# zdule/distributed_learning

Measured on AMD Instinct MI355X. Metric: images/sec (whole node) ResNet-50 synthetic ImageNet, higher is better.
Workload: dtype bf16

## Files before the change

### csrc/include/dla_kernels.h

```cpp
#pragma once

#include <hip/hip_runtime.h>
#include <stdint.h>

#include "dla_dtype.h"
#include "dla_lists.h"

namespace dla {

struct SgdParams {
  float lr;
  float momentum;
  float dampening;
  float weight_decay;
  float grad_scale;
  int nesterov;
  int first_step;
};

void launch_sgd_ema_list(const SgdList& list, const EmaSlots& ema, const float* omd, int nblocks, int grad_dtype,
                         bool use_momentum, const SgdParams& hp, hipStream_t stream);
void launch_ema_update_list(const EmaList& list, int nblocks, const float* omd, hipStream_t stream);
void launch_ema_swap_list(const EmaList& list, int nblocks, hipStream_t stream);
void launch_sgd_list(const SgdList& list, int nblocks, int grad_dtype, bool use_momentum, const SgdParams& hp,
// ... 256 lines not shown
void launch_gemm_nt_splitk(const void* A, int64_t lda, const void* B, int64_t ldb, bool b_kmajor, float* partial,
                           int splits, void* C, int M, int N, int K, const void* addend, int64_t ld_addend,
                           hipStream_t stream);

int conv3x3_stats_rows(int64_t P, int Cout, int tile = kTileAuto, int K = 0, bool wide_ok = true);
int pick_conv_tile(int64_t P, int N, int tile, int K, bool wide_ok);
bool halo_conv_eligible(int Cin, int Cout, int W, int stride, bool fwd);
void launch_conv3x3_halo(const void* x, const void* w, void* y, int N, int H, int W, float* stats,
                         hipStream_t stream, const void* addend = nullptr);
void launch_conv3x3_fwd(const void* x, const void* w, void* y, int N, int H, int W, int Cin, int Cout, int stride,
                        float* stats, hipStream_t stream, int tile = kTileAuto);
void launch_conv3x3_dgrad(const void* dy, const void* w, void* dx, int N, int H, int W, int Cin, int Cout,
                          const void* addend, hipStream_t stream, int tile = kTileAuto,
                          const BnBwdArgs* bn_bwd = nullptr);
void launch_conv3x3s2_dgrad(const void* dy, const void* w, void* dx, int N, int H, int W, int Cin, int Cout,
                            hipStream_t stream);
int stem_stats_rows(int64_t P, int Cout = 64);
int stem_stream_rows(int64_t P, int Cout);
bool launch_stem_stream(const void* xs, const void* wpk, void* y, int N, int BH, int BW, float* stats,
                        hipStream_t stream);
void set_stem_stream(int mode);

void launch_stem_fold(const void* x, void* xs, int N, int H, int W, hipStream_t stream);
void launch_stem_fwd(const void* xs, const void* wpk, void* y, int N, int H, int W, int Cout, float* stats,
                     hipStream_t stream);
int stem_wgrad_splits(int N, int H, int W, int Cout);
void launch_stem_wgrad(const void* dy, const void* xs, float* partial, int splits, void* dwpk, int out_dtype, int N,
                       int H, int W, int Cout, hipStream_t stream);
bool stem_wgrad_bn_eligible(int N, int H, int W, int Cout, int OH, int OW);
int stem_wgrad_bn_splits(int N, int H, int W);
void launch_stem_wgrad_bn(const void* dy_pool, const uint8_t* pos, const void* x, const float* ws, const void* xs,
// ... 13 lines not shown
```

### csrc/include/dla_mfma.h

```cpp
#pragma once

#include "dla_common.h"

namespace dla {
namespace mm {

typedef __bf16 bf16x8_t __attribute__((ext_vector_type(8)));
typedef float f32x4_t __attribute__((ext_vector_type(4)));
typedef short s16x4_t __attribute__((ext_vector_type(4)));

struct FastDiv {
  uint32_t d, m_lo, m_hi;
};
__host__ __device__ inline FastDiv make_fastdiv(uint32_t d) {
  const uint64_t m = ((1ull << 40) + d - 1) / d;
  return FastDiv{d, (uint32_t)m, (uint32_t)(m >> 32)};
}
__device__ __forceinline__ uint32_t fdiv(uint32_t n, const FastDiv& f) {
  return (__umulhi(n, f.m_lo) + n * f.m_hi) >> 8;
}

constexpr int kThreads = 256;
#ifndef DLA_RM_SWIZZLE
#define DLA_RM_SWIZZLE 1
// ... 307 lines not shown
    } else {
      kr = kk * 16 + 8 * (g >> 1) + q;
      cn = r0 + 16 * (g & 1) + 4 * p;
    }
    return tr_frag(s + tr_off<W>(kr, cn), s + tr_off<W>(kr + 4, cn));
  } else {
    if constexpr (DLA_RM_SWIZZLE) {
      const int r = r0 + (lane & (kMS - 1)), lc = kk * (kKS / 8) + lane / kMS;
      return *reinterpret_cast<const bf16x8_t*>(s + r * kBK + ((lc ^ ((r >> 1) & 7)) << 3));
    }
    return *reinterpret_cast<const bf16x8_t*>(s + (r0 + (lane & (kMS - 1))) * (kBK + 8) + kk * kKS +
                                              8 * (lane / kMS));
  }
}

template <int BM, int BN, int NT, bool kT = false, class LA, class LB>
__device__ __forceinline__ void mainloop(const LA& la, const LB& lb, int kbeg, int kend, Acc<BM, BN, NT>& acc,
                                         char* smem) {
  static_assert(LA::kNT == NT && LB::kNT == NT, "loaders built for another block size");
  using GA = TileGeom<BM, NT>;
  using GB = TileGeom<BN, NT>;
  using AC = Acc<BM, BN, NT>;
  constexpr int WM = AC::WM, WN = AC::WN, TM = AC::TM, TN = AC::TN;
  bf16_t* As = reinterpret_cast<bf16_t*>(smem);
  bf16_t* Bs = As + (LA::kKMajor ? GA::kKElems : GA::kRowElems);
  const int wid = threadIdx.x >> 6, wr = wid / AC::WGN, wc = wid % AC::WGN;
  ushort8_t ra[GA::CH], rb[GB::CH];
  auto gload = [&](int k0) {
#pragma unroll
    for (int i = 0; i < GA::CH; ++i) ra[i] = la.load(i, k0);
#pragma unroll
    for (int i = 0; i < GB::CH; ++i) rb[i] = lb.load(i, k0);
  };
  const int nk = (kend - kbeg + kBK - 1) / kBK;
  if (nk <= 0) return;
  gload(kbeg);
  tile_store<BM, LA>(As, ra);
  tile_store<BN, LB>(Bs, rb);
  __syncthreads();
  for (int t = 0; t < nk; ++t) {
    if (t + 1 < nk) gload(kbeg + (t + 1) * kBK);
#pragma unroll
    for (int kk = 0; kk < kBK / kKS; ++kk) {
      bf16x8_t af[TM], bfr[TN];
#pragma unroll
      for (int i = 0; i < TM; ++i) af[i] = tile_frag<BM, LA>(As, wr * WM + i * kMS, kk);
#pragma unroll
      for (int j = 0; j < TN; ++j) bfr[j] = tile_frag<BN, LB>(Bs, wc * WN + j * kMS, kk);
#pragma unroll
      for (int i = 0; i < TM; ++i)
#pragma unroll
        for (int j = 0; j < TN; ++j) acc.v[i][j] = mfma_t<kT>(af[i], bfr[j], acc.v[i][j]);
    }
    __syncthreads();
    if (t + 1 < nk) {
      tile_store<BM, LA>(As, ra);
// ... 8 lines not shown
  const int r = r0 + (lane & (kMS - 1)), lc = kk * (kKS / 8) + lane / kMS;
  return *reinterpret_cast<const bf16x8_t*>(s + r * kBK + ((lc ^ ((r >> 1) & 7)) << 3));
}

template <int W, class L>
__device__ __forceinline__ bf16x8_t glds_frag(const bf16_t* s, int r0, int kk) {
  if constexpr (L::kKMajor) return tile_frag<W, L>(s, r0, kk);
  else return rm_glds_frag(s, r0, kk);
}

template <int BM, int BN, int NS>
__host__ __device__ constexpr size_t glds_lds_bytes() {
  return (size_t)NS * (BM + BN) * kBK * sizeof(bf16_t);
}

template <int BM, int BN, int NT, int NS, bool kT = false, class LA, class LB>
__device__ __forceinline__ void mainloop_glds(const LA& la, const LB& lb, int kbeg, int kend, Acc<BM, BN, NT>& acc,
                                              char* smem) {
  static_assert(NS == 2 || NS == 3, "2 or 3 stages");
  static_assert(LA::kNT == NT && LB::kNT == NT, "loaders built for another block size");
  using GA = TileGeom<BM, NT>;
  using GB = TileGeom<BN, NT>;
  using AC = Acc<BM, BN, NT>;
  constexpr int L = GA::CH + GB::CH;
  constexpr int WM = AC::WM, WN = AC::WN, TM = AC::TM, TN = AC::TN;
  constexpr int SA = BM * kBK, SB = BN * kBK;
  bf16_t* base = reinterpret_cast<bf16_t*>(smem);
  const int wave = threadIdx.x >> 6, wr = wave / AC::WGN, wc = wave % AC::WGN;
  const uint32_t lds0 = lds_addr(smem);
  const uint32_t wofs = (uint32_t)__builtin_amdgcn_readfirstlane(wave * 64 * 16);
  const int nk = (kend - kbeg + kBK - 1) / kBK;
  if (nk <= 0) return;
  LA pa = la;
  LB pb = lb;
  pa.prep();
  pb.prep();
  auto issue = [&](int t) {
    const int st = t % NS;
    const int k0 = kbeg + t * kBK;
    const uint32_t a_base = lds0 + (uint32_t)(st * (SA + SB)) * 2u + wofs;
    const uint32_t b_base = a_base + (uint32_t)SA * 2u;
#pragma unroll
    for (int i = 0; i < GA::CH; ++i) glds16(pa.src(i, k0), a_base + (uint32_t)(i * NT * 16));
#pragma unroll
    for (int i = 0; i < GB::CH; ++i) glds16(pb.src(i, k0), b_base + (uint32_t)(i * NT * 16));
  };
#pragma unroll
  for (int p = 0; p < NS - 1; ++p)
    if (p < nk) issue(p);
  for (int t = 0; t < nk; ++t) {
    if constexpr (NS == 3) {
      if (t + 1 < nk) vm_wait<L>();
      else vm_wait<0>();
    } else {
// ... 46 lines not shown
    bf16x8_t af[TM], bfr[TN];
#pragma unroll
    for (int i = 0; i < TM; ++i) af[i] = glds_frag<BM, LA>(As, wr * WM + i * kMS, kk);
#pragma unroll
    for (int j = 0; j < TN; ++j) bfr[j] = glds_frag<BN, LB>(Bs, wc * WN + j * kMS, kk);
    __builtin_amdgcn_s_setprio(1);
#pragma unroll
    for (int i = 0; i < TM; ++i)
#pragma unroll
      for (int j = 0; j < TN; ++j) acc.v[i][j] = mfma_t<kT>(af[i], bfr[j], acc.v[i][j]);
    __builtin_amdgcn_s_setprio(0);
    if (kk == 0) mid();
  }
}

template <int BM, int BN, int NT, int NS, bool kT = false, class LA, class LB>
__device__ __forceinline__ void mainloop_glds2(const LA& la, const LB& lb, int kbeg, int kend, Acc<BM, BN, NT>& acc,
                                               char* smem) {
  static_assert(NS == 2 || NS == 3, "2 or 3 stages");
  static_assert(LA::kNT == NT && LB::kNT == NT, "loaders built for another block size");
  using GA = TileGeom<BM, NT>;
  using GB = TileGeom<BN, NT>;
  using AC = Acc<BM, BN, NT>;
  constexpr int L = GA::CH + GB::CH;
  constexpr int WM = AC::WM, WN = AC::WN, TM = AC::TM, TN = AC::TN;
  constexpr int SA = BM * kBK, SB = BN * kBK;
  bf16_t* base = reinterpret_cast<bf16_t*>(smem);
  const int wave = threadIdx.x >> 6, wr = wave / AC::WGN, wc = wave % AC::WGN;
  const uint32_t lds0 = lds_addr(smem);
  const uint32_t wofs = (uint32_t)__builtin_amdgcn_readfirstlane(wave * 64 * 16);
  const int nk = (kend - kbeg + kBK - 1) / kBK;
  if (nk <= 0) return;
  LA pa = la;
  LB pb = lb;
  pa.prep();
  pb.prep();
  auto issue_a = [&](int t) {
    const int k0 = kbeg + t * kBK;
    loader_step(pa, k0, 0);
    const uint32_t a_base = lds0 + (uint32_t)((t % NS) * (SA + SB)) * 2u + wofs;
#pragma unroll
    for (int i = 0; i < GA::CH; ++i) glds16(loader_src(pa, i, k0, 0), a_base + (uint32_t)(i * NT * 16));
  };
  auto issue_b = [&](int t) {
    const int k0 = kbeg + t * kBK;
    loader_step(pb, k0, 0);
    const uint32_t b_base = lds0 + (uint32_t)((t % NS) * (SA + SB) + SA) * 2u + wofs;
#pragma unroll
    for (int i = 0; i < GB::CH; ++i) glds16(loader_src(pb, i, k0, 0), b_base + (uint32_t)(i * NT * 16));
  };
#pragma unroll
  for (int p = 0; p < NS - 1; ++p)
    if (p < nk) {
      issue_a(p);
      issue_b(p);
    }
  for (int t = 0; t < nk; ++t) {
    if constexpr (NS == 3) {
      if (t + 1 < nk) vm_wait<L>();
      else vm_wait<0>();
// ... 16 lines not shown

template <class L, int W, int NT>
__device__ __forceinline__ void bissue(const L& l, int k0, uint32_t lds) {
  constexpr int CH = TileGeom<W, NT>::CH;
  uint32_t vo[CH];
  if (l.bcheck(k0)) {
#pragma unroll
    for (int i = 0; i < CH; ++i) vo[i] = l.bvoff_chk(i, k0);
  } else {
#pragma unroll
    for (int i = 0; i < CH; ++i) vo[i] = l.bvo[i];
  }
  bglds<CH, NT * 16>(vo, l.bsrd, (uint32_t)__builtin_amdgcn_readfirstlane(l.bsoff(k0)), lds);
}

template <int BM, int BN, int NT, int NS, bool kT = false, class LA, class LB>
__device__ __forceinline__ void mainloop_bglds(const LA& la, const LB& lb, int kbeg, int kend, Acc<BM, BN, NT>& acc,
                                               char* smem) {
  static_assert(NS == 2 || NS == 3, "2 or 3 stages");
  static_assert(LA::kNT == NT && LB::kNT == NT, "loaders built for another block size");
  using GA = TileGeom<BM, NT>;
  using GB = TileGeom<BN, NT>;
  using AC = Acc<BM, BN, NT>;
  constexpr int L = GA::CH + GB::CH;
  constexpr int WM = AC::WM, WN = AC::WN, TM = AC::TM, TN = AC::TN;
  constexpr int SA = BM * kBK, SB = BN * kBK;
  bf16_t* base = reinterpret_cast<bf16_t*>(smem);
  const int wave = threadIdx.x >> 6, wr = wave / AC::WGN, wc = wave % AC::WGN;
  const uint32_t lds0 = lds_addr(smem);
  const uint32_t wofs = (uint32_t)__builtin_amdgcn_readfirstlane(wave * 64 * 16);
  const int nk = (kend - kbeg + kBK - 1) / kBK;
  if (nk <= 0) return;
  LA pa = la;
  LB pb = lb;
  pa.prep();
  pb.prep();
  pa.bprep();
  pb.bprep();
  auto issue_a = [&](int t) {
    const int k0 = kbeg + t * kBK;
    loader_step(pa, k0, 0);
    bissue<LA, BM, NT>(pa, k0, lds0 + (uint32_t)((t % NS) * (SA + SB)) * 2u + wofs);
  };
  auto issue_b = [&](int t) {
    const int k0 = kbeg + t * kBK;
    loader_step(pb, k0, 0);
    bissue<LB, BN, NT>(pb, k0, lds0 + (uint32_t)((t % NS) * (SA + SB) + SA) * 2u + wofs);
  };
#pragma unroll
  for (int p = 0; p < NS - 1; ++p)
    if (p < nk) {
      issue_a(p);
      issue_b(p);
    }
  for (int t = 0; t < nk; ++t) {
    if constexpr (NS == 3) {
      if (t + 1 < nk) vm_wait<L>();
      else vm_wait<0>();
    } else {
      vm_wait<0>();
    }
    asm volatile("s_waitcnt lgkmcnt(0)" ::: "memory");
    __builtin_amdgcn_s_barrier();
    asm volatile("" ::: "memory");
    const bool more = t + NS - 1 < nk;
    if (more) issue_a(t + NS - 1);
    const bf16_t* As = base + (t % NS) * (SA + SB);
    const bf16_t* Bs = As + SA;
    kstep_mfma<BM, BN, NT, LA, LB, kT>(As, Bs, wr, wc, acc, [&] {
      if (more) issue_b(t + NS - 1);
    });
  }
  __syncthreads();
}

template <int PIPE, bool kT = false, int BM, int BN, int NT, class LA, class LB>
__device__ __forceinline__ void run_mainloop(const LA& la, const LB& lb, int kbeg, int kend, Acc<BM, BN, NT>& acc,
                                             char* smem) {
  if constexpr (PIPE == 0) mainloop<BM, BN, NT, kT>(la, lb, kbeg, kend, acc, smem);
  else if constexpr (PIPE >= 6) mainloop_bglds<BM, BN, NT, PIPE - 4, kT>(la, lb, kbeg, kend, acc, smem);
  else if constexpr (PIPE >= 4) mainloop_glds2<BM, BN, NT, PIPE - 2, kT>(la, lb, kbeg, kend, acc, smem);
  else mainloop_glds<BM, BN, NT, PIPE, kT>(la, lb, kbeg, kend, acc, smem);
}

template <int PIPE, int BM, int BN, class LA, class LB>
__host__ __device__ constexpr size_t run_mainloop_lds_bytes() {
  return PIPE == 0 ? mainloop_lds_bytes<BM, BN, LA, LB>()
                   : glds_lds_bytes<BM, BN, (PIPE >= 6 ? PIPE - 4 : (PIPE >= 4 ? PIPE - 2 : PIPE))>();
}

template <int BM, int BN, bool kStats, int NT = kThreads>
__host__ __device__ constexpr size_t epilogue_lds_bytes() {
  return (size_t)BM * (BN + 8) * sizeof(bf16_t) > (size_t)NT * 64 ? (size_t)BM * (BN + 8) * sizeof(bf16_t)
                                                                  : (size_t)NT * 64;
}

template <int BM, int BN, int NT = kThreads>
// ... 386 lines not shown
```

### csrc/kernels/conv.hip

```cpp
#include "dla_common.h"
#include "dla_kernels.h"
#include "dla_knob.h"
#include "dla_mfma.h"

#include <algorithm>
#include <cstdlib>
#include <type_traits>

namespace dla {

using namespace mm;

struct ConvGeom {
  int N, H, W, Cin;
  int OH, OW, Cout;
  int stride;
  FastDiv fOW, fOH;
};

template <int W, bool kFlip, int NT = kThreads>
struct Im2colRowLoader {
  static constexpr bool kKMajor = false;
  static constexpr int kNT = NT;
  static constexpr int CH = TileGeom<W, NT>::CH;
  const bf16_t* x;
  int H, Wd, C;
// ... 408 lines not shown
  }
  __device__ const void* src(int i, int k0) const {
    const int c = threadIdx.x + i * NT, kr = c / TileGeom<W>::KPR;
    const int p = k0 + kr;
    if (p >= kend || kh[i] < 0) return zero_src();
    const uint32_t q = fdiv((uint32_t)p, g.fOW);
    const int ow = p - (int)q * g.OW;
    const uint32_t n = fdiv(q, g.fOH);
    const int oh = (int)q - (int)n * g.OH;
    const int ih = oh * g.stride - 1 + kh[i], iw = ow * g.stride - 1 + kw[i];
    if ((unsigned)ih >= (unsigned)g.H || (unsigned)iw >= (unsigned)g.W) return zero_src();
    return x + (((int64_t)n * g.H + ih) * g.W + iw) * g.Cin + ci[i];
  }
};

template <int BM, int BN, bool kStats, int PIPE, int NT>
__global__ __launch_bounds__(NT, blocks_per_cu(BM, BN, NT)) void conv3x3_fwd_kernel(const bf16_t* __restrict__ x,
                                                                  const bf16_t* __restrict__ w,
                                                                  bf16_t* __restrict__ y, ConvGeom g,
                                                                  float* __restrict__ stats) {
  extern __shared__ __attribute__((aligned(16))) char smem_raw[];
  const int64_t P = (int64_t)g.N * g.OH * g.OW;
  const int nbn = (g.Cout + BN - 1) / BN;
  const int tile = xcd_remap(blockIdx.x, gridDim.x);
  const int bm = tile / nbn, bn = tile % nbn;
  const int64_t row0 = (int64_t)bm * BM;
  const int col0 = bn * BN;
  const int K = 9 * g.Cin;
  constexpr bool kAny = PIPE >= 100;
  const RowLoader<BN, NT> lb{w, K, (int64_t)col0, g.Cout, K};
  std::conditional_t<kAny, Im2colRowLoaderAnyC<BM, false, NT>, Im2colRowLoader<BM, false, NT>> la{
      x, g.H, g.W, g.Cin, g.stride};
  la.init(g, row0, P, g.OH, g.OW, g.fOW, g.fOH);
  ColStats<BM, BN, NT> st;
  st.zero();
  Acc<BM, BN, NT> acc;
  acc.zero();
  run_mainloop<PIPE % 100>(la, lb, 0, K, acc, smem_raw);
  epilogue_bf16<BM, BN, kStats, false, NT>(acc, y, g.Cout, P, g.Cout, row0, col0, st, nullptr, 0, smem_raw);
  if constexpr (kStats) stats_flush<BM, BN, NT>(st, stats + (int64_t)bm * g.Cout * 2, g.Cout, col0, smem_raw);
}

template <int BM, int BN, int PIPE, int NT>
__global__ __launch_bounds__(NT, blocks_per_cu(BM, BN, NT)) void conv3x3_dgrad_kernel(const bf16_t* __restrict__ dy,
                                                                    const bf16_t* __restrict__ w,
                                                                    bf16_t* __restrict__ dx, ConvGeom g,
                                                                    const bf16_t* __restrict__ addend, BnBwdEpi bnb) {
  extern __shared__ __attribute__((aligned(16))) char smem_raw[];
  const int64_t P = (int64_t)g.N * g.H * g.W;
  const int nbn = (g.Cin + BN - 1) / BN;
  const int tile = xcd_remap(blockIdx.x, gridDim.x);
  const int bm = tile / nbn, bn = tile % nbn;
  const int64_t row0 = (int64_t)bm * BM;
  const int col0 = bn * BN;
  const int K = 9 * g.Cout;
  constexpr bool kAny = PIPE >= 100;
  std::conditional_t<kAny, WeightTapKLoaderAnyC<BN, NT>, WeightTapKLoader<BN, NT>> lb{w, g.Cout, g.Cin, col0};
  if constexpr (kAny) lb.prep();
  std::conditional_t<kAny, Im2colRowLoaderAnyC<BM, true, NT>, Im2colRowLoader<BM, true, NT>> la{dy, g.OH, g.OW,
                                                                                                 g.Cout, 1};
  la.init(g, row0, P, g.H, g.W, g.fOW, g.fOH);
  ColStats<BM, BN, NT> st;
  Acc<BM, BN, NT> acc;
  acc.zero();
  run_mainloop<PIPE % 100>(la, lb, 0, K, acc, smem_raw);
  epilogue_bf16<BM, BN, false, true, NT>(acc, dx, g.Cin, P, g.Cin, row0, col0, st, addend, g.Cin, smem_raw, &bnb, bm);
}

template <int BM, int BN, int PIPE, int NT = kThreads>
__global__ __launch_bounds__(NT, blocks_per_cu(BM, BN, NT)) void conv3x3s2_dgrad_kernel(const bf16_t* __restrict__ dy,
                                                                                      const bf16_t* __restrict__ w,
                                                                                      bf16_t* __restrict__ dx,
                                                                                      ConvGeom g) {
  extern __shared__ __attribute__((aligned(16))) char smem_raw[];
  const int64_t P = (int64_t)g.N * g.OH * g.OW;
  const int nbn = (g.Cin + BN - 1) / BN;
  const int per_class = (int)((P + BM - 1) / BM) * nbn;
  const int cls_slot = blockIdx.x / per_class;
  const S2Class cls{cls_slot < 2 ? 1 : 0, (cls_slot & 1) == 0 ? 1 : 0};
  const int tile = xcd_remap(blockIdx.x - cls_slot * per_class, per_class);
  const int bm = tile / nbn, bn = tile % nbn;
  const int64_t row0 = (int64_t)bm * BM;
  const int col0 = bn * BN;
  const int K = cls.ntaps() * g.Cout;
  const S2WeightKLoader<BN, NT> lb{w, g.Cout, g.Cin, col0, cls};
  S2DgradRowLoader<BM, NT> la{dy, g.OH, g.OW, g.Cout, cls};
  la.init(row0, P, g.fOW, g.fOH);
  ColStats<BM, BN, NT> st;
  Acc<BM, BN, NT> acc;
  acc.zero();
  run_mainloop<PIPE>(la, lb, 0, K, acc, smem_raw);
  const S2RowMap rm{g.OH, g.OW, cls.ph, cls.pw, g.fOW, g.fOH};
  epilogue_bf16<BM, BN, false, false, NT, S2RowMap>(acc, dx, g.Cin, P, g.Cin, row0, col0, st, nullptr, 0,
                                                   smem_raw, nullptr, 0, rm);
}

template <int BM, int BN, int PIPE, int NT = kThreads>
__global__ __launch_bounds__(NT, blocks_per_cu(BM, BN, NT)) void conv3x3_wgrad_kernel(const bf16_t* __restrict__ dy,
                                                                                    const bf16_t* __restrict__ x,
                                                                                    ConvGeom g, float* __restrict__ part,
                                                                                    int k_per_split, int ntiles,
                                                                                    int remap) {
  extern __shared__ __attribute__((aligned(16))) char smem_raw[];
  const int P = g.N * g.OH * g.OW;
  const int Mo = g.Cout, No = 9 * g.Cin;
  const int nbn = (No + BN - 1) / BN;
// ... 31 lines not shown
  g.OH = (H + 2 - 3) / stride + 1;
  g.OW = (W + 2 - 3) / stride + 1;
  g.fOW = make_fastdiv((uint32_t)g.OW);
  g.fOH = make_fastdiv((uint32_t)g.OH);
  return g;
}

template <int BM, int BN, bool S, int PIPE, int NT>
static void launch_fwd_p(const bf16_t* x, const bf16_t* w, bf16_t* y, const ConvGeom& g, float* stats,
                         hipStream_t stream) {
  const int64_t P = (int64_t)g.N * g.OH * g.OW;
  const int tiles = (int)((P + BM - 1) / BM) * ((g.Cout + BN - 1) / BN);
  const size_t lds =
      std::max(run_mainloop_lds_bytes<PIPE % 100, BM, BN, Im2colRowLoader<BM, false, NT>, RowLoader<BN, NT>>(),
               epilogue_lds_bytes<BM, BN, S, NT>());
  hipLaunchKernelGGL((conv3x3_fwd_kernel<BM, BN, S, PIPE, NT>), dim3(tiles), dim3(NT), lds, stream, x, w, y, g,
                     stats);
}
template <int BM, int BN, bool S, int NTW = kThreads>
static void launch_fwd(const bf16_t* x, const bf16_t* w, bf16_t* y, const ConvGeom& g, float* stats,
                       hipStream_t stream) {
  if constexpr (NTW == 512 && BM * BN > 256 * 128) {
    if (mfma_pipeline() == 2) launch_fwd_p<BM, BN, S, 2, 512>(x, w, y, g, stats, stream);
    else launch_fwd_p<BM, BN, S, 6, 512>(x, w, y, g, stats, stream);
  } else if constexpr (NTW == 512) {
    if (mfma_pipeline() == 7) launch_fwd_p<BM, BN, S, 7, 512>(x, w, y, g, stats, stream);
    else launch_fwd_p<BM, BN, S, 3, 512>(x, w, y, g, stats, stream);
  } else if constexpr (BM * BN > 128 * 128) {
    if (mfma_pipeline() == 2) launch_fwd_p<BM, BN, S, 2, kThreads>(x, w, y, g, stats, stream);
    else launch_fwd_p<BM, BN, S, 3, kThreads>(x, w, y, g, stats, stream);
  } else if (g.Cin % 64 != 0) {
    if (mfma_pipeline_for(9 * g.Cin) == 0) launch_fwd_p<BM, BN, S, 100, kThreads>(x, w, y, g, stats, stream);
// ... 49 lines not shown
    case kTile128x64: DLA_CF(128, 64) break;
    default: DLA_CF(64, 64) break;
  }
#undef DLA_CF
#undef DLA_CFW
}

template <int BM, int BN, int PIPE, int NT>
static void launch_dgrad_p(const bf16_t* dy, const bf16_t* w, bf16_t* dx, const ConvGeom& g, const bf16_t* addend,
                           const BnBwdEpi& bnb, hipStream_t stream) {
  const int64_t P = (int64_t)g.N * g.H * g.W;
  const int tiles = (int)((P + BM - 1) / BM) * ((g.Cin + BN - 1) / BN);
  const size_t lds =
      std::max(run_mainloop_lds_bytes<PIPE % 100, BM, BN, Im2colRowLoader<BM, true, NT>, WeightTapKLoader<BN, NT>>(),
               epilogue_lds_bytes<BM, BN, false, NT>());
  hipLaunchKernelGGL((conv3x3_dgrad_kernel<BM, BN, PIPE, NT>), dim3(tiles), dim3(NT), lds, stream, dy, w, dx, g,
                     addend, bnb);
}
template <int BM, int BN, int NTW = kThreads>
static void launch_dgrad(const bf16_t* dy, const bf16_t* w, bf16_t* dx, const ConvGeom& g, const bf16_t* addend,
                         const BnBwdEpi& bnb, hipStream_t stream) {
  if constexpr (NTW == 512 && BM * BN > 256 * 128) {
    if (mfma_pipeline() == 2) launch_dgrad_p<BM, BN, 2, 512>(dy, w, dx, g, addend, bnb, stream);
    else launch_dgrad_p<BM, BN, 6, 512>(dy, w, dx, g, addend, bnb, stream);
  } else if constexpr (NTW == 512) {
    if (mfma_pipeline() == 7) launch_dgrad_p<BM, BN, 7, 512>(dy, w, dx, g, addend, bnb, stream);
    else launch_dgrad_p<BM, BN, 3, 512>(dy, w, dx, g, addend, bnb, stream);
  } else if constexpr (BM * BN > 128 * 128) {
    if (mfma_pipeline() == 2) launch_dgrad_p<BM, BN, 2, kThreads>(dy, w, dx, g, addend, bnb, stream);
    else launch_dgrad_p<BM, BN, 3, kThreads>(dy, w, dx, g, addend, bnb, stream);
  } else if (g.Cout % 64 != 0) {
    if (mfma_pipeline_for(9 * g.Cout) == 0) launch_dgrad_p<BM, BN, 100, kThreads>(dy, w, dx, g, addend, bnb, stream);
// ... 26 lines not shown
  const bf16_t* ad = (const bf16_t*)addend;
  switch (pick_conv_tile((int64_t)N * H * W, Cin, tile, 9 * Cout, Cout % 64 == 0)) {
    case kTile512x128: launch_dgrad<512, 128, 512>(d, wp, (bf16_t*)dx, g, ad, bnb, stream); break;
    case kTile256x256: launch_dgrad<256, 256, 512>(d, wp, (bf16_t*)dx, g, ad, bnb, stream); break;
    case kTile256x128: launch_dgrad<256, 128, 512>(d, wp, (bf16_t*)dx, g, ad, bnb, stream); break;
    case kTile256x128w4: launch_dgrad<256, 128>(d, wp, (bf16_t*)dx, g, ad, bnb, stream); break;
    case kTile128x256w4: launch_dgrad<128, 256>(d, wp, (bf16_t*)dx, g, ad, bnb, stream); break;
    case kTile256x64: launch_dgrad<256, 64>(d, wp, (bf16_t*)dx, g, ad, bnb, stream); break;
    case kTile128x128: launch_dgrad<128, 128>(d, wp, (bf16_t*)dx, g, ad, bnb, stream); break;
    case kTile128x64: launch_dgrad<128, 64>(d, wp, (bf16_t*)dx, g, ad, bnb, stream); break;
    default: launch_dgrad<64, 64>(d, wp, (bf16_t*)dx, g, ad, bnb, stream); break;
  }
}

void launch_conv3x3s2_dgrad(const void* dy, const void* w, void* dx, int N, int H, int W, int Cin, int Cout,
                            hipStream_t stream) {
  const ConvGeom g = make_geom(N, H, W, Cin, Cout, 2);
  const int64_t P = (int64_t)N * g.OH * g.OW;
  if (tile256_enabled() && Cin % 256 == 0 && 4 * ((P + 255) / 256) * (Cin / 256) >= 192) {
    const int pc = (int)((P + 255) / 256) * (Cin / 256);
    hipLaunchKernelGGL((conv3x3s2_dgrad_kernel<256, 256, 2, 512>), dim3(4 * pc), dim3(512),
                       std::max(run_mainloop_lds_bytes<2, 256, 256, S2DgradRowLoader<256, 512>,
                                                       S2WeightKLoader<256, 512>>(),
                                epilogue_lds_bytes<256, 256, false, 512>()),
                       stream, (const bf16_t*)dy, (const bf16_t*)w, (bf16_t*)dx, g);
    return;
  }
  if (tile256_enabled() && tile512_enabled() && Cin == 128 && Cout % 64 == 0 && 4 * ((P + 511) / 512) >= 1024) {
    const int pc = (int)((P + 511) / 512);
    hipLaunchKernelGGL((conv3x3s2_dgrad_kernel<512, 128, 2, 512>), dim3(4 * pc), dim3(512),
                       std::max(run_mainloop_lds_bytes<2, 512, 128, S2DgradRowLoader<512, 512>,
                                                       S2WeightKLoader<128, 512>>(),
                                epilogue_lds_bytes<512, 128, false, 512>()),
                       stream, (const bf16_t*)dy, (const bf16_t*)w, (bf16_t*)dx, g);
    return;
  }
  const int bn = Cin <= 64 ? 64 : 128;
  const int per_class = (int)((P + 127) / 128) * ((Cin + bn - 1) / bn);
#define DLA_S2(BN_, P_)                                                                                          \
  hipLaunchKernelGGL((conv3x3s2_dgrad_kernel<128, BN_, P_>), dim3(4 * per_class), dim3(kThreads),               \
                     std::max(run_mainloop_lds_bytes<P_, 128, BN_, S2DgradRowLoader<128>, S2WeightKLoader<BN_>>(), \
                              epilogue_lds_bytes<128, BN_, false>()),                                           \
                     stream, (const bf16_t*)dy, (const bf16_t*)w, (bf16_t*)dx, g)
  const int pipe = mfma_pipeline_for(4 * Cout);
  if (bn == 64) {
    if (pipe == 0) DLA_S2(64, 0); else DLA_S2(64, 2);
  } else {
    if (pipe == 0) DLA_S2(128, 0); else DLA_S2(128, 2);
  }
#undef DLA_S2
}

static bool wgrad_wide(int Cin, int Cout) { return tn256_enabled() && Cout % 256 == 0 && Cin % 256 == 0; }

static Knob k_wgrad_w4 = Knob::off_unless_1("WGRAD_W4");
// ... 62 lines not shown
```

### csrc/nn_bindings.cpp

```cpp
#include <torch/extension.h>
#include <ATen/hip/HIPContext.h>
#include <c10/hip/HIPStream.h>

#include "dla_bindings.h"
#include "dla_kernels.h"
#include "dla_knob.h"
#include "dla_tables.h"

namespace dla {

static void check_span(const at::Tensor& t, const char* what) {
  int64_t last = 0;
  for (int64_t d = 0; d < t.dim(); ++d) last += (t.size(d) - 1) * t.stride(d);
  const int64_t bytes = t.numel() ? (last + 1) * (int64_t)t.element_size() : 0;
  TORCH_CHECK(bytes < (int64_t(1) << 31), what, ": ", bytes,
              " bytes reach the 2 GiB buffer-descriptor range of the native kernels (lower the per-GPU batch)");
}

static void check_act(const at::Tensor& t, const char* what) {
  TORCH_CHECK(t.is_cuda(), what, " must be a GPU tensor");
  TORCH_CHECK(t.dim() == 4 || t.dim() == 2, what, " must be NCHW-shaped (channels_last) or [M, C]");
  const bool ok = t.dim() == 4 ? t.is_contiguous(at::MemoryFormat::ChannelsLast) : t.is_contiguous();
  TORCH_CHECK(ok, what, " must be channels_last (4-D) or contiguous (2-D)");
  TORCH_CHECK(t.size(1) % 8 == 0, what, ": channel count must be a multiple of 8");
// ... 1003 lines not shown
  at::Tensor dx = dgrad_dx("conv3x3_dgrad", dy, w);
  const int N = (int)dy.size(0), Cout = (int)w.size(0), Cin = (int)w.size(1), H = (int)dy.size(2), W = (int)dy.size(3);
  TORCH_CHECK(Cout % 64 == 0 || tile_bm(tile) * tile_bn(tile) <= 128 * 128,
              "conv3x3_dgrad: Cout % 64 != 0 needs a tile of at most 128x128");
  const void* add = dgrad_addend("conv3x3_dgrad", addend, dx);
  if (tile == 0 && halo_conv_eligible(Cout, Cin, W, 1, false)) {
    const at::Tensor wt = w.flip({2, 3}).transpose(0, 1).contiguous(at::MemoryFormat::ChannelsLast);
    launch_conv3x3_halo(dy.data_ptr(), wt.data_ptr(), dx.data_ptr(), N, H, W, nullptr, current_stream(dy), add);
    return dx;
  }
  launch_conv3x3_dgrad(dy.data_ptr(), w.data_ptr(), dx.data_ptr(), N, H, W, Cin, Cout, add, current_stream(dy),
                       (int)tile);
  return dx;
}

at::Tensor conv3x3s2_dgrad(at::Tensor dy, at::Tensor w, int64_t H, int64_t W) {
  TORCH_CHECK(dy.dim() == 4 && H > 0 && W > 0 && H % 2 == 0 && W % 2 == 0 && dy.size(2) == H / 2 && dy.size(3) == W / 2,
              "conv3x3s2_dgrad: needs even H, W and dy = [N, Cout, H/2, W/2]");
  at::Tensor dx = dgrad_dx("conv3x3s2_dgrad", dy, w, H, W);
  const int N = (int)dy.size(0), Cout = (int)w.size(0), Cin = (int)w.size(1);
  TORCH_CHECK(Cin % 64 == 0 && Cout % 64 == 0, "conv3x3s2_dgrad: Cin and Cout must be multiples of 64");
  launch_conv3x3s2_dgrad(dy.data_ptr(), w.data_ptr(), dx.data_ptr(), N, (int)H, (int)W, Cin, Cout,
                         current_stream(dy));
  return dx;
}

std::vector<at::Tensor> conv3x3_dgrad_bn(at::Tensor dy, at::Tensor w, c10::optional<at::Tensor> addend,
                                         at::Tensor x_bn, at::Tensor ws, c10::optional<at::Tensor> mask, int64_t mode) {
  at::Tensor dx = dgrad_dx("conv3x3_dgrad_bn", dy, w);
  const int N = (int)dy.size(0), Cout = (int)w.size(0), Cin = (int)w.size(1), H = (int)dy.size(2), W = (int)dy.size(3);
  const void* add = dgrad_addend("conv3x3_dgrad_bn", addend, dx);
  const int64_t P = (int64_t)N * H * W;
  at::Tensor part;
  const BnBwdArgs bnb = make_bn_bwd("conv3x3_dgrad_bn", x_bn, ws, mask, mode, P, Cin,
                                    conv3x3_stats_rows(P, Cin, kTileAuto, 9 * Cout, Cout % 64 == 0), part);
  launch_conv3x3_dgrad(dy.data_ptr(), w.data_ptr(), dx.data_ptr(), N, H, W, Cin, Cout, add, current_stream(dy),
                       kTileAuto, &bnb);
  return {dx, part};
// ... 42 lines not shown
        pybind11::arg("M"), pybind11::arg("N"), pybind11::arg("K"), pybind11::arg("lda"), pybind11::arg("ldc"), pybind11::arg("b_kmajor") = false,
        pybind11::arg("add") = false, pybind11::arg("bnb") = false);
  m.def("mfma_pipeline", &mfma_pipeline);
  m.def("set_tile256_min_k_stats", &set_tile256_min_k_stats, "smallest K of the auto 256x256 tiles of statistics forwards (A/B)");
  m.def("set_tile256_min_k", &set_tile256_min_k, "smallest K of the auto 256x256 gemm_nt / conv tiles (A/B; <= 0 default 1024)");
  m.def("set_tn256", &set_tn256, "256x256 weight-gradient tiles: -1 environment (DLA_TN256, default on), 0 off, 1 on");
  m.def("set_splitk_blocks", &set_splitk_blocks, "split-K weight-gradient block target (0 = default / DLA_SPLITK_BLOCKS)");
  m.def("splitk_target_blocks", &splitk_target_blocks);
  m.def("set_bn_red_blocks", &set_bn_red_blocks, "BN reduction-pass block target (0 = default / DLA_BN_RED_BLOCKS)");
  m.def("bn_red_blocks", &bn_red_blocks);
  m.def("conv3x3_fwd", &conv3x3_fwd, "implicit-GEMM 3x3/pad-1 conv forward (NHWC bf16, MFMA)", pybind11::arg("x"),
        pybind11::arg("w"), pybind11::arg("stride") = 1, pybind11::arg("stats") = false, pybind11::arg("tile") = 0);
  m.def("conv3x3_dgrad", &conv3x3_dgrad, "implicit-GEMM 3x3 conv data gradient (stride 1)", pybind11::arg("dy"),
        pybind11::arg("w"), pybind11::arg("addend") = pybind11::none(), pybind11::arg("tile") = 0);
  m.def("conv3x3s2_dgrad", &conv3x3s2_dgrad, "implicit-GEMM 3x3 / stride-2 conv data gradient (parity classes)",
        pybind11::arg("dy"), pybind11::arg("w"), pybind11::arg("H"), pybind11::arg("W"));
  m.def("conv3x3_wgrad", &conv3x3_wgrad, "implicit-GEMM 3x3 conv weight gradient (split-K)", pybind11::arg("dy"),
        pybind11::arg("x"), pybind11::arg("stride") = 1, pybind11::arg("out_dtype") = at::kFloat);
  m.def("bn_relu_maxpool_fwd", &bn_relu_maxpool_fwd, "stem BN(train)+ReLU+max-pool forward (pooled output only)",
        pybind11::arg("x"), pybind11::arg("weight"), pybind11::arg("bias"), pybind11::arg("running_mean"),
        pybind11::arg("running_var"), pybind11::arg("momentum"), pybind11::arg("eps"), pybind11::arg("k"),
        pybind11::arg("s"), pybind11::arg("p"), pybind11::arg("stats") = pybind11::none(),
        pybind11::arg("ceil_mode") = false);
  m.def("bn_relu_maxpool_bwd", &bn_relu_maxpool_bwd, "stem BN+ReLU+max-pool backward (dy gathered from the pool)",
        pybind11::arg("dy_pool"), pybind11::arg("pos"), pybind11::arg("x"), pybind11::arg("ws"), pybind11::arg("weight"),
        pybind11::arg("k"), pybind11::arg("s"), pybind11::arg("p"), pybind11::arg("want_dx") = true);
  m.def("maxpool_fwd", &maxpool_fwd, "NHWC max pooling forward (+ argmax window positions)", pybind11::arg("x"),
        pybind11::arg("k"), pybind11::arg("s"), pybind11::arg("p"), pybind11::arg("ceil_mode") = false,
        pybind11::arg("need_pos") = true);
  m.def("maxpool_bwd", &maxpool_bwd, "NHWC max pooling backward (gather form)");
  m.def("set_pool3_sep", &set_pool3_sep, "3x3/s1 max-pool forward: 4 / 7-row separable strips, 0 generic kernel, -1 environment (default 4)");
// ... 98 lines not shown
```

Before: 16040.

## Iterate 3x3 conv GEMM K loop tap-major within channel chunks

Adds a pluggable K-step mapping to the MFMA mainloops and uses it in the 3x3 conv forward, dgrad and stride-2 dgrad kernels. The K loop then visits all taps for one channel chunk before moving to the next chunk, instead of walking the taps linearly. This is meant to improve cache locality of the im2col input and weight loads, since neighbouring taps reuse overlapping input rows. It also adds an optional class-minor block ordering for the stride-2 dgrad and an explicit tile override in the binding. A compile-time bitmask selects which kernel families use the new ordering, and it adds some index arithmetic per K step.

```diff
diff --git a/csrc/include/dla_kernels.h b/csrc/include/dla_kernels.h
--- a/csrc/include/dla_kernels.h
+++ b/csrc/include/dla_kernels.h
@@ -294,7 +294,7 @@
                           const void* addend, hipStream_t stream, int tile = kTileAuto,
                           const BnBwdArgs* bn_bwd = nullptr);
 void launch_conv3x3s2_dgrad(const void* dy, const void* w, void* dx, int N, int H, int W, int Cin, int Cout,
-                            hipStream_t stream);
+                            hipStream_t stream, int tile = kTileAuto);
 int stem_stats_rows(int64_t P, int Cout = 64);
 int stem_stream_rows(int64_t P, int Cout);
 bool launch_stem_stream(const void* xs, const void* wpk, void* y, int N, int BH, int BW, float* stats,
diff --git a/csrc/include/dla_mfma.h b/csrc/include/dla_mfma.h
--- a/csrc/include/dla_mfma.h
+++ b/csrc/include/dla_mfma.h
@@ -345,9 +345,13 @@
   }
 }
 
-template <int BM, int BN, int NT, bool kT = false, class LA, class LB>
+struct KStepLinear {
+  __device__ __forceinline__ int operator()(int kbeg, int t) const { return kbeg + t * kBK; }
+};
+
+template <int BM, int BN, int NT, bool kT = false, class LA, class LB, class KM = KStepLinear>
 __device__ __forceinline__ void mainloop(const LA& la, const LB& lb, int kbeg, int kend, Acc<BM, BN, NT>& acc,
-                                         char* smem) {
+                                         char* smem, const KM& km = KM()) {
   static_assert(LA::kNT == NT && LB::kNT == NT, "loaders built for another block size");
   using GA = TileGeom<BM, NT>;
   using GB = TileGeom<BN, NT>;
@@ -365,12 +369,12 @@
   };
   const int nk = (kend - kbeg + kBK - 1) / kBK;
   if (nk <= 0) return;
-  gload(kbeg);
+  gload(km(kbeg, 0));
   tile_store<BM, LA>(As, ra);
   tile_store<BN, LB>(Bs, rb);
   __syncthreads();
   for (int t = 0; t < nk; ++t) {
-    if (t + 1 < nk) gload(kbeg + (t + 1) * kBK);
+    if (t + 1 < nk) gload(km(kbeg, t + 1));
 #pragma unroll
     for (int kk = 0; kk < kBK / kKS; ++kk) {
       bf16x8_t af[TM], bfr[TN];
@@ -409,9 +413,9 @@
   return (size_t)NS * (BM + BN) * kBK * sizeof(bf16_t);
 }
 
-template <int BM, int BN, int NT, int NS, bool kT = false, class LA, class LB>
+template <int BM, int BN, int NT, int NS, bool kT = false, class LA, class LB, class KM = KStepLinear>
 __device__ __forceinline__ void mainloop_glds(const LA& la, const LB& lb, int kbeg, int kend, Acc<BM, BN, NT>& acc,
-                                              char* smem) {
+                                              char* smem, const KM& km = KM()) {
   static_assert(NS == 2 || NS == 3, "2 or 3 stages");
   static_assert(LA::kNT == NT && LB::kNT == NT, "loaders built for another block size");
   using GA = TileGeom<BM, NT>;
@@ -432,7 +436,7 @@
   pb.prep();
   auto issue = [&](int t) {
     const int st = t % NS;
-    const int k0 = kbeg + t * kBK;
+    const int k0 = km(kbeg, t);
     const uint32_t a_base = lds0 + (uint32_t)(st * (SA + SB)) * 2u + wofs;
     const uint32_t b_base = a_base + (uint32_t)SA * 2u;
 #pragma unroll
@@ -509,9 +513,9 @@
   }
 }
 
-template <int BM, int BN, int NT, int NS, bool kT = false, class LA, class LB>
+template <int BM, int BN, int NT, int NS, bool kT = false, class LA, class LB, class KM = KStepLinear>
 __device__ __forceinline__ void mainloop_glds2(const LA& la, const LB& lb, int kbeg, int kend, Acc<BM, BN, NT>& acc,
-                                               char* smem) {
+                                               char* smem, const KM& km = KM()) {
   static_assert(NS == 2 || NS == 3, "2 or 3 stages");
   static_assert(LA::kNT == NT && LB::kNT == NT, "loaders built for another block size");
   using GA = TileGeom<BM, NT>;
@@ -531,14 +535,14 @@
   pa.prep();
   pb.prep();
   auto issue_a = [&](int t) {
-    const int k0 = kbeg + t * kBK;
+    const int k0 = km(kbeg, t);
     loader_step(pa, k0, 0);
     const uint32_t a_base = lds0 + (uint32_t)((t % NS) * (SA + SB)) * 2u + wofs;
 #pragma unroll
     for (int i = 0; i < GA::CH; ++i) glds16(loader_src(pa, i, k0, 0), a_base + (uint32_t)(i * NT * 16));
   };
   auto issue_b = [&](int t) {
-    const int k0 = kbeg + t * kBK;
+    const int k0 = km(kbeg, t);
     loader_step(pb, k0, 0);
     const uint32_t b_base = lds0 + (uint32_t)((t % NS) * (SA + SB) + SA) * 2u + wofs;
 #pragma unroll
@@ -585,9 +589,9 @@
   bglds<CH, NT * 16>(vo, l.bsrd, (uint32_t)__builtin_amdgcn_readfirstlane(l.bsoff(k0)), lds);
 }
 
-template <int BM, int BN, int NT, int NS, bool kT = false, class LA, class LB>
+template <int BM, int BN, int NT, int NS, bool kT = false, class LA, class LB, class KM = KStepLinear>
 __device__ __forceinline__ void mainloop_bglds(const LA& la, const LB& lb, int kbeg, int kend, Acc<BM, BN, NT>& acc,
-                                               char* smem) {
+                                               char* smem, const KM& km = KM()) {
   static_assert(NS == 2 || NS == 3, "2 or 3 stages");
   static_assert(LA::kNT == NT && LB::kNT == NT, "loaders built for another block size");
   using GA = TileGeom<BM, NT>;
@@ -609,12 +613,12 @@
   pa.bprep();
   pb.bprep();
   auto issue_a = [&](int t) {
-    const int k0 = kbeg + t * kBK;
+    const int k0 = km(kbeg, t);
     loader_step(pa, k0, 0);
     bissue<LA, BM, NT>(pa, k0, lds0 + (uint32_t)((t % NS) * (SA + SB)) * 2u + wofs);
   };
   auto issue_b = [&](int t) {
-    const int k0 = kbeg + t * kBK;
+    const int k0 = km(kbeg, t);
     loader_step(pb, k0, 0);
     bissue<LB, BN, NT>(pb, k0, lds0 + (uint32_t)((t % NS) * (SA + SB) + SA) * 2u + wofs);
   };
@@ -645,13 +649,13 @@
   __syncthreads();
 }
 
-template <int PIPE, bool kT = false, int BM, int BN, int NT, class LA, class LB>
+template <int PIPE, bool kT = false, int BM, int BN, int NT, class LA, class LB, class KM = KStepLinear>
 __device__ __forceinline__ void run_mainloop(const LA& la, const LB& lb, int kbeg, int kend, Acc<BM, BN, NT>& acc,
-                                             char* smem) {
-  if constexpr (PIPE == 0) mainloop<BM, BN, NT, kT>(la, lb, kbeg, kend, acc, smem);
-  else if constexpr (PIPE >= 6) mainloop_bglds<BM, BN, NT, PIPE - 4, kT>(la, lb, kbeg, kend, acc, smem);
-  else if constexpr (PIPE >= 4) mainloop_glds2<BM, BN, NT, PIPE - 2, kT>(la, lb, kbeg, kend, acc, smem);
-  else mainloop_glds<BM, BN, NT, PIPE, kT>(la, lb, kbeg, kend, acc, smem);
+                                             char* smem, const KM& km = KM()) {
+  if constexpr (PIPE == 0) mainloop<BM, BN, NT, kT>(la, lb, kbeg, kend, acc, smem, km);
+  else if constexpr (PIPE >= 6) mainloop_bglds<BM, BN, NT, PIPE - 4, kT>(la, lb, kbeg, kend, acc, smem, km);
+  else if constexpr (PIPE >= 4) mainloop_glds2<BM, BN, NT, PIPE - 2, kT>(la, lb, kbeg, kend, acc, smem, km);
+  else mainloop_glds<BM, BN, NT, PIPE, kT>(la, lb, kbeg, kend, acc, smem, km);
 }
 
 template <int PIPE, int BM, int BN, class LA, class LB>
diff --git a/csrc/kernels/conv.hip b/csrc/kernels/conv.hip
--- a/csrc/kernels/conv.hip
+++ b/csrc/kernels/conv.hip
@@ -10,6 +10,29 @@
 namespace dla {
 
 using namespace mm;
+
+#ifndef DLA_CONV_KORDER
+#define DLA_CONV_KORDER 191
+#endif
+enum KOrderUse : int { kKoFwd = 1, kKoDgrad = 8, kKoS2 = 64, kKoS2Blocks = 512 };
+constexpr bool conv_korder(int use, int BM, int BN) {
+  const int fam = (BM == 256 && BN == 256) ? 0 : (BM == 512 && BN == 128) ? 1 : 2;
+  return ((DLA_CONV_KORDER) & (use << fam)) != 0;
+}
+
+struct KStepTap9 {
+  int C;
+  __device__ __forceinline__ int operator()(int, int t) const {
+    const int chunk = t / 9;
+    return (t - 9 * chunk) * C + chunk * kBK;
+  }
+};
+struct KStepTapPow2 {
+  int C, lg;
+  __device__ __forceinline__ int operator()(int, int t) const {
+    return (t & ((1 << lg) - 1)) * C + (t >> lg) * kBK;
+  }
+};
 
 struct ConvGeom {
   int N, H, W, Cin;
@@ -448,7 +471,7 @@
   }
 };
 
-template <int BM, int BN, bool kStats, int PIPE, int NT>
+template <int BM, int BN, bool kStats, int PIPE, int NT, bool kTapK>
 __global__ __launch_bounds__(NT, blocks_per_cu(BM, BN, NT)) void conv3x3_fwd_kernel(const bf16_t* __restrict__ x,
                                                                   const bf16_t* __restrict__ w,
                                                                   bf16_t* __restrict__ y, ConvGeom g,
@@ -470,12 +493,13 @@
   st.zero();
   Acc<BM, BN, NT> acc;
   acc.zero();
-  run_mainloop<PIPE % 100>(la, lb, 0, K, acc, smem_raw);
+  if constexpr (kTapK && !kAny) run_mainloop<PIPE % 100>(la, lb, 0, K, acc, smem_raw, KStepTap9{g.Cin});
+  else run_mainloop<PIPE % 100>(la, lb, 0, K, acc, smem_raw);
   epilogue_bf16<BM, BN, kStats, false, NT>(acc, y, g.Cout, P, g.Cout, row0, col0, st, nullptr, 0, smem_raw);
   if constexpr (kStats) stats_flush<BM, BN, NT>(st, stats + (int64_t)bm * g.Cout * 2, g.Cout, col0, smem_raw);
 }
 
-template <int BM, int BN, int PIPE, int NT>
+template <int BM, int BN, int PIPE, int NT, bool kTapK>
 __global__ __launch_bounds__(NT, blocks_per_cu(BM, BN, NT)) void conv3x3_dgrad_kernel(const bf16_t* __restrict__ dy,
                                                                     const bf16_t* __restrict__ w,
                                                                     bf16_t* __restrict__ dx, ConvGeom g,
@@ -497,11 +521,12 @@
   ColStats<BM, BN, NT> st;
   Acc<BM, BN, NT> acc;
   acc.zero();
-  run_mainloop<PIPE % 100>(la, lb, 0, K, acc, smem_raw);
+  if constexpr (kTapK && !kAny) run_mainloop<PIPE % 100>(la, lb, 0, K, acc, smem_raw, KStepTap9{g.Cout});
+  else run_mainloop<PIPE % 100>(la, lb, 0, K, acc, smem_raw);
   epilogue_bf16<BM, BN, false, true, NT>(acc, dx, g.Cin, P, g.Cin, row0, col0, st, addend, g.Cin, smem_raw, &bnb, bm);
 }
 
-template <int BM, int BN, int PIPE, int NT = kThreads>
+template <int BM, int BN, int PIPE, int NT, bool kTapK, bool kClsMinor>
 __global__ __launch_bounds__(NT, blocks_per_cu(BM, BN, NT)) void conv3x3s2_dgrad_kernel(const bf16_t* __restrict__ dy,
                                                                                       const bf16_t* __restrict__ w,
                                                                                       bf16_t* __restrict__ dx,
@@ -510,9 +535,16 @@
   const int64_t P = (int64_t)g.N * g.OH * g.OW;
   const int nbn = (g.Cin + BN - 1) / BN;
   const int per_class = (int)((P + BM - 1) / BM) * nbn;
-  const int cls_slot = blockIdx.x / per_class;
+  int cls_slot, tile;
+  if constexpr (kClsMinor) {
+    const int lin = xcd_remap(blockIdx.x, 4 * per_class);
+    cls_slot = lin & 3;
+    tile = lin >> 2;
+  } else {
+    cls_slot = blockIdx.x / per_class;
+    tile = xcd_remap(blockIdx.x - cls_slot * per_class, per_class);
+  }
   const S2Class cls{cls_slot < 2 ? 1 : 0, (cls_slot & 1) == 0 ? 1 : 0};
-  const int tile = xcd_remap(blockIdx.x - cls_slot * per_class, per_class);
   const int bm = tile / nbn, bn = tile % nbn;
   const int64_t row0 = (int64_t)bm * BM;
   const int col0 = bn * BN;
@@ -523,7 +555,8 @@
   ColStats<BM, BN, NT> st;
   Acc<BM, BN, NT> acc;
   acc.zero();
-  run_mainloop<PIPE>(la, lb, 0, K, acc, smem_raw);
+  if constexpr (kTapK) run_mainloop<PIPE>(la, lb, 0, K, acc, smem_raw, KStepTapPow2{g.Cout, cls.ph + cls.pw});
+  else run_mainloop<PIPE>(la, lb, 0, K, acc, smem_raw);
   const S2RowMap rm{g.OH, g.OW, cls.ph, cls.pw, g.fOW, g.fOH};
   epilogue_bf16<BM, BN, false, false, NT, S2RowMap>(acc, dx, g.Cin, P, g.Cin, row0, col0, st, nullptr, 0,
                                                    smem_raw, nullptr, 0, rm);
@@ -585,8 +618,8 @@
   const size_t lds =
       std::max(run_mainloop_lds_bytes<PIPE % 100, BM, BN, Im2colRowLoader<BM, false, NT>, RowLoader<BN, NT>>(),
                epilogue_lds_bytes<BM, BN, S, NT>());
-  hipLaunchKernelGGL((conv3x3_fwd_kernel<BM, BN, S, PIPE, NT>), dim3(tiles), dim3(NT), lds, stream, x, w, y, g,
-                     stats);
+  hipLaunchKernelGGL((conv3x3_fwd_kernel<BM, BN, S, PIPE, NT, PIPE < 100 && conv_korder(kKoFwd, BM, BN)>), dim3(tiles),
+                     dim3(NT), lds, stream, x, w, y, g, stats);
 }
 template <int BM, int BN, bool S, int NTW = kThreads>
 static void launch_fwd(const bf16_t* x, const bf16_t* w, bf16_t* y, const ConvGeom& g, float* stats,
@@ -666,8 +699,8 @@
   const size_t lds =
       std::max(run_mainloop_lds_bytes<PIPE % 100, BM, BN, Im2colRowLoader<BM, true, NT>, WeightTapKLoader<BN, NT>>(),
                epilogue_lds_bytes<BM, BN, false, NT>());
-  hipLaunchKernelGGL((conv3x3_dgrad_kernel<BM, BN, PIPE, NT>), dim3(tiles), dim3(NT), lds, stream, dy, w, dx, g,
-                     addend, bnb);
+  hipLaunchKernelGGL((conv3x3_dgrad_kernel<BM, BN, PIPE, NT, PIPE < 100 && conv_korder(kKoDgrad, BM, BN)>), dim3(tiles),
+                     dim3(NT), lds, stream, dy, w, dx, g, addend, bnb);
 }
 template <int BM, int BN, int NTW = kThreads>
 static void launch_dgrad(const bf16_t* dy, const bf16_t* w, bf16_t* dx, const ConvGeom& g, const bf16_t* addend,
@@ -724,21 +757,28 @@
 }
 
 void launch_conv3x3s2_dgrad(const void* dy, const void* w, void* dx, int N, int H, int W, int Cin, int Cout,
-                            hipStream_t stream) {
+                            hipStream_t stream, int tile) {
   const ConvGeom g = make_geom(N, H, W, Cin, Cout, 2);
   const int64_t P = (int64_t)N * g.OH * g.OW;
-  if (tile256_enabled() && Cin % 256 == 0 && 4 * ((P + 255) / 256) * (Cin / 256) >= 192) {
+  const bool autot = tile == kTileAuto;
+  if (autot ? tile256_enabled() && Cin % 256 == 0 && 4 * ((P + 255) / 256) * (Cin / 256) >= 192
+            : tile == kTile256x256) {
     const int pc = (int)((P + 255) / 256) * (Cin / 256);
-    hipLaunchKernelGGL((conv3x3s2_dgrad_kernel<256, 256, 2, 512>), dim3(4 * pc), dim3(512),
+    hipLaunchKernelGGL((conv3x3s2_dgrad_kernel<256, 256, 2, 512, conv_korder(kKoS2, 256, 256),
+                                               conv_korder(kKoS2Blocks, 256, 256)>),
+                       dim3(4 * pc), dim3(512),
                        std::max(run_mainloop_lds_bytes<2, 256, 256, S2DgradRowLoader<256, 512>,
                                                        S2WeightKLoader<256, 512>>(),
                                 epilogue_lds_bytes<256, 256, false, 512>()),
                        stream, (const bf16_t*)dy, (const bf16_t*)w, (bf16_t*)dx, g);
     return;
   }
-  if (tile256_enabled() && tile512_enabled() && Cin == 128 && Cout % 64 == 0 && 4 * ((P + 511) / 512) >= 1024) {
+  if (autot ? tile256_enabled() && tile512_enabled() && Cin == 128 && Cout % 64 == 0 && 4 * ((P + 511) / 512) >= 1024
+            : tile == kTile512x128) {
     const int pc = (int)((P + 511) / 512);
-    hipLaunchKernelGGL((conv3x3s2_dgrad_kernel<512, 128, 2, 512>), dim3(4 * pc), dim3(512),
+    hipLaunchKernelGGL((conv3x3s2_dgrad_kernel<512, 128, 2, 512, conv_korder(kKoS2, 512, 128),
+                                               conv_korder(kKoS2Blocks, 512, 128)>),
+                       dim3(4 * pc), dim3(512),
                        std::max(run_mainloop_lds_bytes<2, 512, 128, S2DgradRowLoader<512, 512>,
                                                        S2WeightKLoader<128, 512>>(),
                                 epilogue_lds_bytes<512, 128, false, 512>()),
@@ -748,7 +788,9 @@
   const int bn = Cin <= 64 ? 64 : 128;
   const int per_class = (int)((P + 127) / 128) * ((Cin + bn - 1) / bn);
 #define DLA_S2(BN_, P_)                                                                                          \
-  hipLaunchKernelGGL((conv3x3s2_dgrad_kernel<128, BN_, P_>), dim3(4 * per_class), dim3(kThreads),               \
+  hipLaunchKernelGGL((conv3x3s2_dgrad_kernel<128, BN_, P_, kThreads, conv_korder(kKoS2, 128, BN_),               \
+                                             conv_korder(kKoS2Blocks, 128, BN_)>),                             \
+                     dim3(4 * per_class), dim3(kThreads),                                                        \
                      std::max(run_mainloop_lds_bytes<P_, 128, BN_, S2DgradRowLoader<128>, S2WeightKLoader<BN_>>(), \
                               epilogue_lds_bytes<128, BN_, false>()),                                           \
                      stream, (const bf16_t*)dy, (const bf16_t*)w, (bf16_t*)dx, g)
diff --git a/csrc/nn_bindings.cpp b/csrc/nn_bindings.cpp
--- a/csrc/nn_bindings.cpp
+++ b/csrc/nn_bindings.cpp
@@ -1041,14 +1041,17 @@
   return dx;
 }
 
-at::Tensor conv3x3s2_dgrad(at::Tensor dy, at::Tensor w, int64_t H, int64_t W) {
+at::Tensor conv3x3s2_dgrad(at::Tensor dy, at::Tensor w, int64_t H, int64_t W, int64_t tile) {
   TORCH_CHECK(dy.dim() == 4 && H > 0 && W > 0 && H % 2 == 0 && W % 2 == 0 && dy.size(2) == H / 2 && dy.size(3) == W / 2,
               "conv3x3s2_dgrad: needs even H, W and dy = [N, Cout, H/2, W/2]");
   at::Tensor dx = dgrad_dx("conv3x3s2_dgrad", dy, w, H, W);
   const int N = (int)dy.size(0), Cout = (int)w.size(0), Cin = (int)w.size(1);
   TORCH_CHECK(Cin % 64 == 0 && Cout % 64 == 0, "conv3x3s2_dgrad: Cin and Cout must be multiples of 64");
+  TORCH_CHECK(tile == kTileAuto || tile == kTile128x128 || (tile == kTile256x256 && Cin % 256 == 0) ||
+                  (tile == kTile512x128 && Cin == 128),
+              "conv3x3s2_dgrad: tile 0 (auto), 1 (128 rows), 8 (256x256, Cin % 256 == 0) or 9 (512x128, Cin == 128)");
   launch_conv3x3s2_dgrad(dy.data_ptr(), w.data_ptr(), dx.data_ptr(), N, (int)H, (int)W, Cin, Cout,
-                         current_stream(dy));
+                         current_stream(dy), (int)tile);
   return dx;
 }
 
@@ -1121,7 +1124,7 @@
   m.def("conv3x3_dgrad", &conv3x3_dgrad, "implicit-GEMM 3x3 conv data gradient (stride 1)", pybind11::arg("dy"),
         pybind11::arg("w"), pybind11::arg("addend") = pybind11::none(), pybind11::arg("tile") = 0);
   m.def("conv3x3s2_dgrad", &conv3x3s2_dgrad, "implicit-GEMM 3x3 / stride-2 conv data gradient (parity classes)",
-        pybind11::arg("dy"), pybind11::arg("w"), pybind11::arg("H"), pybind11::arg("W"));
+        pybind11::arg("dy"), pybind11::arg("w"), pybind11::arg("H"), pybind11::arg("W"), pybind11::arg("tile") = 0);
   m.def("conv3x3_wgrad", &conv3x3_wgrad, "implicit-GEMM 3x3 conv weight gradient (split-K)", pybind11::arg("dy"),
         pybind11::arg("x"), pybind11::arg("stride") = 1, pybind11::arg("out_dtype") = at::kFloat);
   m.def("bn_relu_maxpool_fwd", &bn_relu_maxpool_fwd, "stem BN(train)+ReLU+max-pool forward (pooled output only)",
```

Result: no change. 15900 (-0.9%).
